# leochlon/aecf

Hardware: AMD Instinct MI355X
Metric: fused samples/sec (fwd+bwd) (higher is better)
Workload: dtype bf16; 1 GPU; c2: [B=65536 per GPU, M=3, d=512, 8 heads] mask_prob=0.15 train-mode curriculum masking, fwd+bwd; global_batch=65536, parallelism=dp1, world_size=1

## Files before the change

aecf_amd/csrc/aecf_gemm_ws.hip:

```cpp
#include <stdlib.h>

#include "aecf_kernels.h"
#include "aecf_tile.h"

namespace aecf {

namespace {

enum { WS_PLAIN = 0, WS_VPROJ = 1, WS_VFLAT = 2 };

constexpr int WS_PF = 3, VPROJ_PF = 3, DX_PF = 3;

constexpr int ws_plain_bufs(int, int) { return 2; }

template <int KT, int NROWS, int KEYDIV>
__device__ __forceinline__ void ws_dma_rows(const char* __restrict__ src, unsigned int ld_bytes, int rows_valid, char* lds) {
    constexpr int CPR = 4 * KT;
    constexpr int TOTAL = NROWS * CPR;
    constexpr int NI = (TOTAL + 511) / 512;
    static_assert(TOTAL % 64 == 0, "whole wave-instructions");
    const int wbase = __builtin_amdgcn_readfirstlane((int)(threadIdx.x & ~63u));
#pragma unroll
    for (int i = 0; i < NI; ++i) {
        if (wbase + 512 * i < TOTAL) {
            const int c = threadIdx.x + 512 * i;
            const int row = c / CPR, p = c - row * CPR;
            const int rowc = row < rows_valid ? row : rows_valid - 1;
            const int key = (row / KEYDIV) & 15;
            const unsigned int voff = (unsigned)rowc * ld_bytes + (unsigned)((p ^ key) << 4);
            __builtin_amdgcn_global_load_lds(src + voff, (lds_void_t*)(lds + (wbase + 512 * i) * 16), 16, 0, 0);
        }
    }
}

template <int CT>
__device__ __forceinline__ void store_packed(unsigned short* dst, const unsigned int* pk) {
    if (CT == 2) *reinterpret_cast<u32x4*>(dst) = u32x4{pk[0], pk[1], pk[2], pk[3]};
    else *reinterpret_cast<u32x2*>(dst) = u32x2{pk[0], pk[1]};
}
template <int CT>
__device__ __forceinline__ void store_cols_f32(float* dst, const float* v) {
    *reinterpret_cast<f32x4*>(dst) = f32x4{v[0], v[1], v[2], v[3]};
    if (CT == 2) *reinterpret_cast<f32x4*>(dst + 4) = f32x4{v[4], v[5], v[6], v[7]};
}
template <int CT>
__device__ __forceinline__ void store_cols(unsigned short* dst, const float* v);
template <int CT>
__device__ __forceinline__ void store_cols_lo(unsigned short* dst, const float* v) {
    float lo[4 * CT];
#pragma unroll
    for (int j = 0; j < 4 * CT; ++j) lo[j] = v[j] - Tr<BF16>::to_f32(Tr<BF16>::from_f32(v[j]));
    store_cols<CT>(dst, lo);
}
template <int CT>
__device__ __forceinline__ void store_cols(unsigned short* dst, const float* v) {
    if (CT == 2) {
        *reinterpret_cast<u32x4*>(dst) = u32x4{pack_bf16x2(v[0], v[1]), pack_bf16x2(v[2], v[3]), pack_bf16x2(v[4], v[5]),
// ... 10 lines not shown
    for (int m = 0; m < M_; ++m) {
        sc[m] = __builtin_amdgcn_exp2f((sc[m] - mx) * 1.44269504088896340736f);
        sum += sc[m];
    }
    float inv = __builtin_amdgcn_rcpf(sum);
    inv = inv * (2.0f - sum * inv);
#pragma unroll
    for (int m = 0; m < M_; ++m) sc[m] *= inv;
}

template <int NV>
__device__ __forceinline__ void load_bias(const unsigned short* bs, int col, float* bias) {
#pragma unroll
    for (int j = 0; j < NV; ++j) bias[j] = 0.f;
    if (bs) {
        if (NV == 8) {
            Tr<BF16>::unpack(*reinterpret_cast<const u32x4*>(bs + col), bias);
        } else {
            Tr<BF16>::load4(bs + col, bias);
        }
    }
}

template <int KT, int MODE, int M_, bool GATE, int CT>
__global__ __launch_bounds__(512, 2) void gemm_ws_kernel(GemmNtArgs p, int rows_per_block, int nchunk) {
    using X = Tr<BF16>;
    constexpr int K = 32 * KT, ROWB = 2 * K;
    constexpr bool PL = MODE != WS_VPROJ;
    constexpr bool VF = MODE == WS_VFLAT;
    constexpr int NPM = MODE == WS_VPROJ ? M_ : (VF ? 2 : 1);
    constexpr int RT = PL ? 2 : M_;
    constexpr int SROWS = 16 * RT;
    constexpr int OROWS = PL ? 32 : 16;
    constexpr int TILE = SROWS * ROWB;
    constexpr int NBUF = ws_plain_bufs(MODE, KT);
    constexpr int NI_DMA = SROWS * 4 * KT / 512;
    extern __shared__ __attribute__((aligned(16))) char smem[];

    const int lane = lane_id(), r16 = lane & 15, lg = lane >> 4, w = wave_id();
    const int N = p.N, H = p.H;
    unsigned int chunk_u, group_u;
    constexpr int CW = 16 * CT, BC = 8 * CW, NV = 4 * CT;
    if (!xcd_tile(blockIdx.x, (unsigned)nchunk, (unsigned)(p.N / BC), chunk_u, group_u)) return;
    const int ncol0 = (int)group_u * BC + CW * w;
    const int64_t o_beg = (int64_t)chunk_u * rows_per_block;
    const int64_t o_all = p.R;
    const int64_t o_end = (o_beg + rows_per_block) < o_all ? (o_beg + rows_per_block) : o_all;
// ... 21 lines not shown

    const unsigned short* wsrc = reinterpret_cast<const unsigned short*>(p.w);
    u32x4 wreg[KT][CT];
#pragma unroll
    for (int c = 0; c < CT; ++c) {
        const int n = CT == 2 ? ncol0 + 8 * (r16 >> 2) + 4 * c + (r16 & 3) : ncol0 + r16;
        const unsigned short* wr = wsrc + (int64_t)n * K + 8 * lg;
        const u32x4* wf = reinterpret_cast<const u32x4*>(p.w_frag) + ((int64_t)((ncol0 / CW) * CT + c) * KT) * 64 + lane;
#pragma unroll
        for (int ks = 0; ks < KT; ++ks) wreg[ks][c] = p.w_frag ? wf[ks * 64] : *reinterpret_cast<const u32x4*>(wr + 32 * ks);
    }
    float bias[NV];
    load_bias<NV>(reinterpret_cast<const unsigned short*>(p.bias), ncol0 + NV * lg, bias);
    const int head = ncol0 / p.hd;

    int xaddr[4];
#pragma unroll
    for (int v = 0; v < 4; ++v)
        xaddr[v] = (PL ? r16 : r16 * M_) * ROWB + ((((4 * v) + lg) ^ r16) << 4);

    float pm[NPM], pm_next[NPM];
    constexpr int KG = (KT + 7) / 8;
    float* gpart = reinterpret_cast<float*>(smem + 2 * TILE);
    u32x4 ga[GATE ? KG : 1][2];
    if (GATE) {
#pragma unroll
        for (int kg = 0; kg < KG; ++kg) {
            const int ks = KG * w + kg;
            const unsigned short* ah = reinterpret_cast<const unsigned short*>(p.g_ahi) + (int64_t)r16 * K + 32 * ks + 8 * lg;
            const unsigned short* al = reinterpret_cast<const unsigned short*>(p.g_alo) + (int64_t)r16 * K + 32 * ks + 8 * lg;
            ga[kg][0] = ks < KT ? *reinterpret_cast<const u32x4*>(ah) : u32x4{0u, 0u, 0u, 0u};
            ga[kg][1] = ks < KT ? *reinterpret_cast<const u32x4*>(al) : u32x4{0u, 0u, 0u, 0u};
        }
    }
    unsigned int kp[GATE ? M_ : 1], kp_next[GATE ? M_ : 1];
    auto load_probs = [&](int64_t o0, float* dst) {
        if (MODE == WS_VPROJ && GATE) {
            if (p.g_kpm) {
                const int64_t b = (o0 + r16) < o_end ? (o0 + r16) : (o_end - 1);
                const uint8_t* kq = p.g_kpm + b * M_;
#pragma unroll
                for (int m = 0; m < M_; ++m)
                    asm volatile("global_load_ubyte %0, %1, off" : "=v"(kp_next[m]) : "v"(kq + m) : "memory");
            }
        } else if (MODE == WS_VPROJ) {
            const int64_t b = (o0 + r16) < o_end ? (o0 + r16) : (o_end - 1);
            const float* pp = p.probs + (b * H + head) * M_;
#pragma unroll
            for (int m = 0; m < M_; ++m)
                asm volatile("global_load_dword %0, %1, off" : "=v"(dst[m]) : "v"(pp + m) : "memory");
        } else if (VF) {
#pragma unroll
            for (int t = 0; t < 2; ++t) {
                const int64_t row = (o0 + 16 * t + r16) < o_end ? (o0 + 16 * t + r16) : (o_end - 1);
// ... 10 lines not shown
        if (GATE) { asm volatile("" : "+v"(kp_next[m])); kp[m] = p.g_kpm ? kp_next[m] : 0u; }
        else asm volatile("" : "+v"(pm[m]));
    }
    int cur = 0;
    for (int64_t o0 = o_beg; o0 < o_end; o0 += OROWS, cur = (cur + 1 == NBUF ? 0 : cur + 1)) {
        __builtin_amdgcn_s_barrier();
        const bool two_ahead = NBUF == 3 && o0 + 2 * OROWS < o_end;
        if (NBUF == 3) { if (two_ahead) issue(o0 + 2 * OROWS, cur >= 1 ? cur - 1 : 2); }
        else if (!GATE && o0 + OROWS < o_end) issue(o0 + OROWS, cur ^ 1);
        if (o0 + OROWS < o_end) load_probs(o0 + OROWS, pm_next);

        if (GATE) {
            const char* tg = smem + cur * TILE;
            f32x4 gacc[M_];
#pragma unroll
            for (int m = 0; m < M_; ++m) {
                gacc[m] = f32x4{0.f, 0.f, 0.f, 0.f};
#pragma unroll
                for (int kg = 0; kg < KG; ++kg) {
                    const int ks = (KG * w + kg) % KT;
                    const int xo = r16 * M_ * ROWB + m * ROWB + ((((ks & 3) * 4 + lg) ^ r16) << 4) + (ks >> 2) * 256;
                    const u32x4 xf = *reinterpret_cast<const u32x4*>(tg + xo);
                    gacc[m] = X::mma(ga[kg][0], xf, gacc[m]);
                    gacc[m] = X::mma(ga[kg][1], xf, gacc[m]);
                }
#pragma unroll
                for (int r = 0; r < 4; ++r) gpart[((w * M_ + m) * 16 + 4 * lg + r) * 16 + r16] = gacc[m][r];
            }
            asm volatile("s_waitcnt lgkmcnt(0)" ::: "memory");
            __builtin_amdgcn_s_barrier();
            float sc[M_], mx = -INFINITY;
#pragma unroll
            for (int m = 0; m < M_; ++m) {
                float a = 0.f;
#pragma unroll
                for (int ww = 0; ww < 8; ++ww) a += gpart[((ww * M_ + m) * 16 + head) * 16 + r16];
                if (kp[m] != 0u) a = -INFINITY;
                sc[m] = a;
                mx = fmaxf(mx, a);
            }
            softmax_fast<M_>(sc, mx);
            const int64_t bq = o0 + r16;
            const bool writer = lg == 0 && ncol0 % p.hd == 0 && bq < o_end;
#pragma unroll
            for (int m = 0; m < M_; ++m) pm[m] = sc[m];
            if (writer) {
                float* dst = const_cast<float*>(p.probs) + (bq * H + head) * M_;
#pragma unroll
                for (int m = 0; m < M_; ++m) dst[m] = pm[m];
            }
        }

        constexpr int NIT = RT * KT;
        constexpr int PF = WS_PF;
        const char* tb = smem + cur * TILE;
        auto rd = [&](int i) -> u32x4 {
            const int ks = PL ? i / RT : i % KT;
            const int t = PL ? i % RT : i / KT;
            const int toff = (PL ? 16 * t * ROWB : t * ROWB) + (ks >> 2) * 256;
            return *reinterpret_cast<const u32x4*>(tb + xaddr[ks & 3] + toff);
        };
        constexpr int NACC = PL ? RT : 1;
        f32x4 acc[NACC][CT];
#pragma unroll
        for (int t = 0; t < NACC; ++t)
#pragma unroll
            for (int c = 0; c < CT; ++c) acc[t][c] = f32x4{0.f, 0.f, 0.f, 0.f};
        float ov[NV];
        unsigned int vpk[MODE == WS_VPROJ ? M_ : 1][NV / 2];
#pragma unroll
        for (int j = 0; j < NV; ++j) ov[j] = 0.f;

        u32x4 xf[PF + 1];
#pragma unroll
        for (int i = 0; i < PF; ++i) xf[i] = rd(i);
        __builtin_amdgcn_sched_group_barrier(0x100, PF, 0);
#pragma unroll
        for (int i = 0; i < NIT; ++i) {
            if (i + PF < NIT) xf[(i + PF) % (PF + 1)] = rd(i + PF);
            if (GATE && i == NIT / 8 && o0 + OROWS < o_end) issue(o0 + OROWS, cur ^ 1);
            const int ks = PL ? i / RT : i % KT;
            const int t = PL ? i % RT : 0;
#pragma unroll
            for (int c = 0; c < CT; ++c) acc[t][c] = X::mma(wreg[ks][c], xf[i % (PF + 1)], acc[t][c]);
            __builtin_amdgcn_sched_group_barrier(0x100, 1, 0);
            __builtin_amdgcn_sched_group_barrier(0x008, CT, 0);
            if (MODE == WS_VPROJ && ks == KT - 1) {
                const int m = i / KT;
                float v[NV];
#pragma unroll
                for (int c = 0; c < CT; ++c)
#pragma unroll
                    for (int r = 0; r < 4; ++r) {
                        v[4 * c + r] = acc[0][c][r] + bias[4 * c + r];
                        ov[4 * c + r] = fmaf(pm[m], v[4 * c + r], ov[4 * c + r]);
                    }
#pragma unroll
                for (int j = 0; j < NV / 2; ++j) vpk[m][j] = pack_bf16x2(v[2 * j], v[2 * j + 1]);
#pragma unroll
                for (int c = 0; c < CT; ++c) acc[0][c] = f32x4{0.f, 0.f, 0.f, 0.f};
            }
        }

        if (two_ahead) asm volatile("s_waitcnt vmcnt(%0)" ::"n"(NI_DMA) : "memory");
        else asm volatile("s_waitcnt vmcnt(0)" ::: "memory");
        float pm_now[NPM];
#pragma unroll
        for (int m = 0; m < NPM; ++m) pm_now[m] = pm[m];
#pragma unroll
        for (int m = 0; m < NPM; ++m) {
            if (GATE) {
                asm volatile("" : "+v"(kp_next[m]));
                kp[m] = p.g_kpm ? kp_next[m] : 0u;
            } else {
                asm volatile("" : "+v"(pm_next[m]));
                pm[m] = pm_next[m];
            }
        }
        if (PL) {
#pragma unroll
            for (int t = 0; t < RT; ++t) {
// ... 9 lines not shown
                        else store_cols<CT>(reinterpret_cast<unsigned short*>(p.c) + row * N + ncol0 + NV * lg, v);
                        if (p.c_lo) store_cols_lo<CT>(reinterpret_cast<unsigned short*>(p.c_lo) + row * N + ncol0 + NV * lg, v);
                    }
                } else {
                    if (p.v_out && row < o_end)
                        store_cols<CT>(reinterpret_cast<unsigned short*>(p.v_out) + row * N + ncol0 + NV * lg, v);
                    float ow[NV];
#pragma unroll
                    for (int j = 0; j < NV; ++j) {
                        float a = pm_now[t] * v[j];
                        a += __shfl_xor(a, 1, 64);
                        a += __shfl_xor(a, 2, 64);
                        ow[j] = a;
                    }
                    if ((r16 & 3) == 0 && row < o_end) {
                        store_cols<CT>(reinterpret_cast<unsigned short*>(p.c) + (row / M_) * N + ncol0 + NV * lg, ow);
                        if (p.c_lo) store_cols_lo<CT>(reinterpret_cast<unsigned short*>(p.c_lo) + (row / M_) * N + ncol0 + NV * lg, ow);
                    }
                }
            }
        } else {
            const int64_t b = o0 + r16;
            if (b < o_end) {
                if (p.v_out) {
#pragma unroll
                    for (int m = 0; m < M_; ++m)
                        store_packed<CT>(reinterpret_cast<unsigned short*>(p.v_out) + (b * M_ + m) * N + ncol0 + NV * lg, vpk[m]);
                }
                if (p.out_f32) store_cols_f32<CT>(reinterpret_cast<float*>(p.c) + b * N + ncol0 + NV * lg, ov);
                else store_cols<CT>(reinterpret_cast<unsigned short*>(p.c) + b * N + ncol0 + NV * lg, ov);
                if (p.c_lo) store_cols_lo<CT>(reinterpret_cast<unsigned short*>(p.c_lo) + b * N + ncol0 + NV * lg, ov);
            }
        }
    }
}

template <int KT, int HK, int M_, int CT>
__global__ __launch_bounds__(512, 2) void dx_ws2_kernel(BwdGArgs p, int rows_per_block, int nchunk) {
    using X = Tr<BF16>;
    constexpr int CW = 16 * CT, BC = 8 * CW, NV = 4 * CT;
    constexpr int K = 32 * KT, ROWB = 2 * K;
    constexpr int H_ = KT / HK;
    constexpr int KX = (3 * H_ + 31) / 32;
    constexpr int RAW = 16 * ROWB;
    constexpr int HM = H_ * M_, NST = 16 * HM;
    constexpr int HMS = HM | 1;
    extern __shared__ __attribute__((aligned(16))) char smem[];
    constexpr int XROWB = 64 * KX + 16;
    constexpr int XT = 16 * M_ * XROWB;
    char* raw = smem;
// ... 193 lines not shown
    }
}

template <int KT, int HK, int M_, bool HILO>
__global__ __launch_bounds__(512, 2) void dsu_ws_kernel(BwdGArgs p, float* __restrict__ u_slab, int rows_per_block, int nchunk) {
    using X = Tr<BF16>;
    constexpr int KJ = 8;
    constexpr int E = 32 * KT, JB = 32 * KJ, NCT = KT / 4;
    constexpr int HBL = KJ / HK;
    constexpr int ROWX = 2 * E, ROWD = 2 * JB;
    constexpr int XROWS = 16 * M_;
    constexpr int KU = (XROWS + 31) / 32;
    constexpr int ZROWS = (32 * KU - XROWS) > 0 ? 1 : 0;
    constexpr int PSTR = HBL * M_ * 16;
    constexpr int DSROW = 72;
    constexpr int XT = XROWS * ROWX, DT = 16 * ROWD;
    constexpr int NPART = 8;
    extern __shared__ __attribute__((aligned(16))) char smem[];
    char* xb = smem;
    char* zp = smem + 2 * XT;
    char* db = zp + ZROWS * ROWX;
    char* dbl = db + 2 * DT;
    float* part = reinterpret_cast<float*>(db + (HILO ? 4 : 2) * DT);
    unsigned short* dsh = reinterpret_cast<unsigned short*>(reinterpret_cast<char*>(part) + NPART * PSTR * 4);
    unsigned short* dsl = dsh + 16 * DSROW;

    const int lane = lane_id(), r16 = lane & 15, lg = lane >> 4;
    const int w = __builtin_amdgcn_readfirstlane(wave_id());
    const int H = p.H;
    unsigned int chunk_u, group_u;
    if (!xcd_tile(blockIdx.x, (unsigned)nchunk, (unsigned)(E / JB), chunk_u, group_u)) return;
    const int jbase = (int)group_u * JB, hbase = jbase / (32 * HK);
    const int ncol0 = 16 * NCT * w;
    const int64_t o_beg = (int64_t)chunk_u * rows_per_block;
    const int64_t o_end = (o_beg + rows_per_block) < p.B ? (o_beg + rows_per_block) : p.B;
    if (o_beg >= o_end) return;

    const char* dsrc = reinterpret_cast<const char*>(p.dobuf) + (int64_t)jbase * 2;
    const char* xsrc = reinterpret_cast<const char*>(p.x);
    const char* dlsrc = HILO ? reinterpret_cast<const char*>(p.do_lo) + (int64_t)jbase * 2 : dsrc;
    auto issue = [&](int64_t o0, int buf) {
        const int ov = (int)((o_end - o0) < 16 ? (o_end - o0) : 16);
        ws_dma_rows_asm<KT, 16 * M_, M_>(xsrc + o0 * M_ * (int64_t)ROWX, (unsigned)ROWX, ov * M_, xb + buf * XT);
        ws_dma_rows_asm<KJ, 16, 1>(dsrc + o0 * (int64_t)ROWX, (unsigned)ROWX, ov, db + buf * DT);
        if (HILO) ws_dma_rows_asm<KJ, 16, 1>(dlsrc + o0 * (int64_t)ROWX, (unsigned)ROWX, ov, dbl + buf * DT);
    };
    for (int i = threadIdx.x; i < ZROWS * ROWX / 16; i += 512) reinterpret_cast<u32x4*>(zp)[i] = u32x4{0u, 0u, 0u, 0u};
    for (int i = threadIdx.x; i < 2 * 16 * DSROW / 2; i += 512) reinterpret_cast<unsigned int*>(dsh)[i] = 0u;
    issue(o_beg, 0);

    const unsigned short* wsrc = reinterpret_cast<const unsigned short*>(p.wvt);
    u32x4 wreg[KJ][NCT];
    static_assert(NCT % 2 == 0, "tile pairs");
#pragma unroll
    for (int ct = 0; ct < NCT; ++ct) {
        const int krow = ncol0 + 32 * (ct >> 1) + 8 * (r16 >> 2) + 4 * (ct & 1) + (r16 & 3);
        const unsigned short* wr = wsrc + (int64_t)krow * E + jbase + 8 * lg;
#pragma unroll
        for (int ks = 0; ks < KJ; ++ks) wreg[ks][ct] = *reinterpret_cast<const u32x4*>(wr + 32 * ks);
    }
    int daddr[4];
#pragma unroll
    for (int v = 0; v < 4; ++v) daddr[v] = r16 * ROWD + ((((4 * v) + lg) ^ r16) << 4);
    const int xaddr0 = r16 * M_ * ROWX + ((((ncol0 >> 3) + lg) ^ r16) << 4);
    const int q = r16 >> 2, pp = r16 & 3;
    int ua[KU][2];
    bool uz[KU][2];
#pragma unroll
    for (int ks = 0; ks < KU; ++ks) {
#pragma unroll
        for (int hh = 0; hh < 2; ++hh) {
// ... 102 lines not shown
            if (ds_m < M_) {
                const float* pr = part + (ds_hh * M_ + ds_m) * 16 + ds_s;
#pragma unroll
                for (int i = 0; i < NPART; ++i) da += pr[i * PSTR];
            }
            float dw = p.d_attn_w ? dwb : 0.f;
            if (p.d_entropy && ds_m < M_) {
                int64_t be = o0 + ds_s;
                be = be < o_end ? be : o_end - 1;
                float hsum = 0.f;
#pragma unroll
                for (int m = 0; m < M_; ++m) hsum -= xlogx(p.attn_w[be * M_ + m]);
                const bool live = (hsum >= 0.f) && (hsum <= p.log_M);
                dw += live ? -(logf(p.attn_w[be * M_ + ds_m]) + 1.0f) * p.d_entropy[be] : 0.f;
            }
            const float dp = da + dw * invH;
            const float dot = reduce_lg((ds_m < M_) ? pmv * dp : 0.f);
            const int64_t b = o0 + ds_s;
            if (ds_m < M_) {
                const float d = (b < o_end) ? pmv * (dp - dot) : 0.f;
                if (b < o_end) p.dsbuf[(b * H + hbase + ds_hh) * M_ + ds_m] = d;
                const unsigned short hi = X::from_f32(d);
                dsh[ds_hh * DSROW + kslot(ds_s, ds_m)] = hi;
                dsl[ds_hh * DSROW + kslot(ds_s, ds_m)] = X::from_f32(d - X::to_f32(hi));
            }
        }
        asm volatile("s_waitcnt lgkmcnt(0)" ::: "memory");
        __builtin_amdgcn_s_barrier();
#pragma unroll
        for (int ks = 0; ks < KU; ++ks) {
            const u32x4 bh = *reinterpret_cast<const u32x4*>(reinterpret_cast<const char*>(dsh) + (r16 * DSROW + 32 * ks + 8 * lg) * 2);
            const u32x4 bl = *reinterpret_cast<const u32x4*>(reinterpret_cast<const char*>(dsl) + (r16 * DSROW + 32 * ks + 8 * lg) * 2);
#pragma unroll
            for (int ct = 0; ct < NCT; ++ct) {
                const u32x4 af = tr_frag16(smem, (uz[ks][0] ? 0 : cur * XT) + (ua[ks][0] ^ (32 * ct)),
                                           (uz[ks][1] ? 0 : cur * XT) + (ua[ks][1] ^ (32 * ct)));
                uacc[ct] = X::mma(af, bh, uacc[ct]);
                uacc[ct] = X::mma(af, bl, uacc[ct]);
            }
        }
        asm volatile("s_waitcnt vmcnt(0)" ::: "memory");
        asm volatile("" : "+v"(pmv_n), "+v"(dwb_n));
        pmv = pmv_n; dwb = dwb_n;
    }
    if (r16 < HBL) {
#pragma unroll
        for (int ct = 0; ct < NCT; ++ct)
            *reinterpret_cast<f32x4*>(u_slab + ((int64_t)chunk_u * H + hbase + r16) * E + ncol0 + 16 * ct + 4 * lg) = uacc[ct];
    }
}


static size_t dsu_ws_smem(int E, int M, int hd, bool lo) {
    constexpr int JB = 256;
    const int xrows = 16 * M, zrows = (32 * ((xrows + 31) / 32) - xrows) > 0 ? 1 : 0, hbl = JB / hd;
    return (size_t)(2 * xrows + zrows) * 2 * E + (size_t)(lo ? 4 : 2) * 16 * 2 * JB + (size_t)8 * (16 * hbl * M) * 4 +
           (size_t)2 * 16 * 72 * 2;
}

template <int KT, int HK, int M_>
int launch_dsu_t(const BwdGArgs& a, float* u_slab, hipStream_t s) {
    constexpr int E = 32 * KT, JB = 256;
    const bool hilo = a.do_lo && dsu_ws_takes_lo(a);
    const size_t smem = dsu_ws_smem(E, M_, a.hd, hilo);
    const int groups = E / JB;
    int64_t chunks = 256 / groups;
    if (chunks < 1) chunks = 1;
    int64_t rpb = (a.B + chunks - 1) / chunks;
    rpb = (rpb + 15) / 16 * 16;
    const int64_t nchunk = (a.B + rpb - 1) / rpb;
    dim3 grid(xcd_grid((unsigned)nchunk, (unsigned)groups)), block(512);
    if constexpr (!(E == 512 && M_ == 4)) {
        if (hilo) {
            auto kern = dsu_ws_kernel<KT, HK, M_, true>;
            (void)hipFuncSetAttribute(reinterpret_cast<const void*>(kern), hipFuncAttributeMaxDynamicSharedMemorySize, (int)smem);
            kern<<<grid, block, smem, s>>>(a, u_slab, (int)rpb, (int)nchunk);
            return (int)nchunk;
        }
    }
    auto kern = dsu_ws_kernel<KT, HK, M_, false>;
// ... 30 lines not shown
        default: launch_dx2<KT, HK, 4>(a, s); break;
    }
}

template <int KT>
bool launch_dx2_hk(const BwdGArgs& a, hipStream_t s) {
    static_assert(KT % 8 == 0 && KT <= 32, "K = 256, 512, 768, 1024");
    const int hk = a.hd / 32;
    if (hk * a.H != KT) return false;
    if constexpr (KT <= 16) {
        if (hk == 1) { launch_dx2_m<KT, 1>(a, s); return true; }
    }
    if (hk == 2) { launch_dx2_m<KT, 2>(a, s); return true; }
    if constexpr (KT % 3 == 0) {
        if (hk == 3) { launch_dx2_m<KT, 3>(a, s); return true; }
    }
    if (hk == 4) { launch_dx2_m<KT, 4>(a, s); return true; }
    if (hk == 8) { launch_dx2_m<KT, 8>(a, s); return true; }
    if (hk == KT) { launch_dx2_m<KT, KT>(a, s); return true; }
    return false;
}


template <int M_>
__global__ __launch_bounds__(512, 2) void vproj_slab_kernel(GemmNtArgs p, int rows_per_block, int nchunk) {
    using X = Tr<BF16>;
    constexpr int KT = 16, K = 512, CT = 2, KG = 2;
    constexpr int SB = 128;
    constexpr int SLAB = 16 * M_ * SB;
    constexpr int TILE = 8 * SLAB;
    constexpr int CW = 32, BC = 256, NV = 8;
    constexpr int GP = 8 * M_ * 256;
    constexpr int NDMA = 16 * M_ * SB / 1024;
    extern __shared__ __attribute__((aligned(16))) char smem[];
    float* gpart = reinterpret_cast<float*>(smem + 2 * TILE);

    const int lane = lane_id(), r16 = lane & 15, lg = lane >> 4;
    const int w = __builtin_amdgcn_readfirstlane(wave_id());
    const int N = p.N, H = p.H;
    unsigned int chunk_u, group_u;
    if (!xcd_tile(blockIdx.x, (unsigned)nchunk, (unsigned)(p.N / BC), chunk_u, group_u)) return;
    const int ncol0 = (int)group_u * BC + CW * w;
    const int64_t o_beg = (int64_t)chunk_u * rows_per_block;
    const int64_t o_end = (o_beg + rows_per_block) < p.R ? (o_beg + rows_per_block) : p.R;
    if (o_beg >= o_end) return;

    const char* asrc = reinterpret_cast<const char*>(p.a);
    const unsigned int row_pitch = (unsigned)K * 2u;
    auto issue_piece = [&](int64_t o0, int buf, int i) {
        const int ov = (int)((o_end - o0) < 16 ? (o_end - o0) : 16);
        const char* src = asrc + o0 * M_ * (int64_t)row_pitch + SB * w;
        const int rho = 8 * i + (lane >> 3), m = rho >> 4, b = rho & 15;
        const int bc = b < ov ? b : ov - 1;
        const unsigned int voff = (unsigned)(bc * M_ + m) * row_pitch + (unsigned)(((lane & 7) ^ (b & 7)) << 4);
        const unsigned int dst = (unsigned)(size_t)(lds_void_t*)(smem + buf * TILE + w * SLAB + 1024 * i);
// ... 6 lines not shown
    auto issue = [&](int64_t o0, int buf) {
#pragma unroll
        for (int i = 0; i < NDMA; ++i) issue_piece(o0, buf, i);
    };
    issue(o_beg, 0);

    const unsigned short* wsrc = reinterpret_cast<const unsigned short*>(p.w);
    u32x4 wreg[KT][CT];
#pragma unroll
    for (int c = 0; c < CT; ++c) {
        const int n = ncol0 + 8 * (r16 >> 2) + 4 * c + (r16 & 3);
        const unsigned short* wr = wsrc + (int64_t)n * K + 8 * lg;
        const u32x4* wf = reinterpret_cast<const u32x4*>(p.w_frag) + ((int64_t)((ncol0 / CW) * CT + c) * KT) * 64 + lane;
#pragma unroll
        for (int ks = 0; ks < KT; ++ks) wreg[ks][c] = p.w_frag ? wf[ks * 64] : *reinterpret_cast<const u32x4*>(wr + 32 * ks);
    }
    float bias[NV];
    load_bias<NV>(reinterpret_cast<const unsigned short*>(p.bias), ncol0 + NV * lg, bias);
    const int head = ncol0 / p.hd;
    int xoff[KG];
#pragma unroll
    for (int kk = 0; kk < KG; ++kk) xoff[kk] = r16 * SB + ((((4 * kk) + lg) ^ (r16 & 7)) << 4);

    u32x4 ga[KG][2];
#pragma unroll
    for (int kg = 0; kg < KG; ++kg) {
        const int ks = KG * w + kg;
        ga[kg][0] = *reinterpret_cast<const u32x4*>(reinterpret_cast<const unsigned short*>(p.g_ahi) + (int64_t)r16 * K + 32 * ks + 8 * lg);
        ga[kg][1] = *reinterpret_cast<const u32x4*>(reinterpret_cast<const unsigned short*>(p.g_alo) + (int64_t)r16 * K + 32 * ks + 8 * lg);
    }
    unsigned int kp[M_], kp_next[M_];
    {
        const int64_t b0 = (o_beg + r16) < o_end ? (o_beg + r16) : (o_end - 1);
#pragma unroll
        for (int m = 0; m < M_; ++m) {
            kp[m] = p.g_kpm ? (unsigned int)p.g_kpm[b0 * M_ + m] : 0u;
            kp_next[m] = 0u;
        }
    }
    auto load_kp = [&](int64_t o0) {
        if (p.g_kpm) {
            const int64_t b = (o0 + r16) < o_end ? (o0 + r16) : (o_end - 1);
            const uint8_t* kq = p.g_kpm + b * M_;
#pragma unroll
            for (int m = 0; m < M_; ++m) asm volatile("global_load_ubyte %0, %1, off" : "+v"(kp_next[m]) : "v"(kq + m) : "memory");
        }
    };
    auto scores = [&](int buf, float* gp) {
        const char* sl = smem + buf * TILE + w * SLAB;
#pragma unroll
        for (int m = 0; m < M_; ++m) {
            f32x4 gacc = f32x4{0.f, 0.f, 0.f, 0.f};
#pragma unroll
            for (int kg = 0; kg < KG; ++kg) {
                const u32x4 xf = *reinterpret_cast<const u32x4*>(sl + m * 16 * SB + xoff[kg]);
                gacc = X::mma(ga[kg][0], xf, gacc);
                gacc = X::mma(ga[kg][1], xf, gacc);
            }
#pragma unroll
            for (int r = 0; r < 4; ++r) gp[((w * M_ + m) * 16 + 4 * lg + r) * 16 + r16] = gacc[r];
        }
    };
#pragma unroll
    for (int ks = 0; ks < KT; ++ks)
#pragma unroll
        for (int c = 0; c < CT; ++c) asm volatile("" : "+v"(wreg[ks][c]));
#pragma unroll
    for (int kg = 0; kg < KG; ++kg) asm volatile("" : "+v"(ga[kg][0]), "+v"(ga[kg][1]));
    asm volatile("s_waitcnt vmcnt(0)" ::: "memory");
    scores(0, gpart);

    int cur = 0;
    for (int64_t o0 = o_beg; o0 < o_end; o0 += 16, cur ^= 1) {
        const bool more = o0 + 16 < o_end;
        asm volatile("s_waitcnt lgkmcnt(0)" ::: "memory");
        __builtin_amdgcn_s_barrier();
        if (more) load_kp(o0 + 16);
        float pm[M_];
        {
            const float* gp = gpart + cur * GP;
            float mx = -INFINITY;
#pragma unroll
            for (int m = 0; m < M_; ++m) {
                float a = 0.f;
#pragma unroll
                for (int ww = 0; ww < 8; ++ww) a += gp[((ww * M_ + m) * 16 + head) * 16 + r16];
                if (kp[m] != 0u) a = -INFINITY;
                pm[m] = a;
                mx = fmaxf(mx, a);
            }
            softmax_fast<M_>(pm, mx);
            const int64_t bq = o0 + r16;
            const bool writer = lg == 0 && ncol0 % p.hd == 0 && bq < o_end;
            if (writer) {
                float* dst = const_cast<float*>(p.probs) + (bq * H + head) * M_;
#pragma unroll
                for (int m = 0; m < M_; ++m) dst[m] = pm[m];
            }
        }
        constexpr int NIT = M_ * KT, PF = VPROJ_PF;
        const char* tb = smem + cur * TILE;
        auto rd = [&](int i) -> u32x4 {
            const int ks = i % KT, m = i / KT;
            return *reinterpret_cast<const u32x4*>(tb + (ks >> 1) * SLAB + m * 16 * SB + xoff[ks & 1]);
        };
        f32x4 acc[CT];
#pragma unroll
        for (int c = 0; c < CT; ++c) acc[c] = f32x4{0.f, 0.f, 0.f, 0.f};
        float ov[NV];
        unsigned int vpk[M_][NV / 2];
#pragma unroll
        for (int j = 0; j < NV; ++j) ov[j] = 0.f;
        u32x4 xf[PF + 1];
#pragma unroll
        for (int i = 0; i < PF; ++i) xf[i] = rd(i);
        __builtin_amdgcn_sched_group_barrier(0x100, PF, 0);
#pragma unroll
        for (int i = 0; i < NIT; ++i) {
            if (i + PF < NIT) xf[(i + PF) % (PF + 1)] = rd(i + PF);
            if (i == NIT / 8 && more) issue(o0 + 16, cur ^ 1);
            const int ks = i % KT;
#pragma unroll
            for (int c = 0; c < CT; ++c) acc[c] = X::mma(wreg[ks][c], xf[i % (PF + 1)], acc[c]);
            __builtin_amdgcn_sched_group_barrier(0x100, 1, 0);
            __builtin_amdgcn_sched_group_barrier(0x008, CT, 0);
            if (ks == KT - 1) {
                const int m = i / KT;
                float v[NV];
#pragma unroll
                for (int c = 0; c < CT; ++c)
#pragma unroll
                    for (int r = 0; r < 4; ++r) {
                        v[4 * c + r] = acc[c][r] + bias[4 * c + r];
                        ov[4 * c + r] = fmaf(pm[m], v[4 * c + r], ov[4 * c + r]);
                    }
#pragma unroll
                for (int j = 0; j < NV / 2; ++j) vpk[m][j] = pack_bf16x2(v[2 * j], v[2 * j + 1]);
#pragma unroll
                for (int c = 0; c < CT; ++c) acc[c] = f32x4{0.f, 0.f, 0.f, 0.f};
            }
        }
        asm volatile("s_waitcnt vmcnt(0)" ::: "memory");
#pragma unroll
        for (int m = 0; m < M_; ++m) { asm volatile("" : "+v"(kp_next[m])); kp[m] = p.g_kpm ? kp_next[m] : 0u; }
        if (more) scores(cur ^ 1, gpart + (cur ^ 1) * GP);
        const int64_t b = o0 + r16;
        if (b < o_end) {
            if (p.v_out) {
#pragma unroll
                for (int m = 0; m < M_; ++m)
                    store_packed<CT>(reinterpret_cast<unsigned short*>(p.v_out) + (b * M_ + m) * N + ncol0 + NV * lg, vpk[m]);
            }
            if (p.out_f32) store_cols_f32<CT>(reinterpret_cast<float*>(p.c) + b * N + ncol0 + NV * lg, ov);
            else store_cols<CT>(reinterpret_cast<unsigned short*>(p.c) + b * N + ncol0 + NV * lg, ov);
            if (p.c_lo) store_cols_lo<CT>(reinterpret_cast<unsigned short*>(p.c_lo) + b * N + ncol0 + NV * lg, ov);
        }
    }
}

template <int M_>
void launch_vproj_slab(const GemmNtArgs& a, hipStream_t s) {
    const size_t smem = (size_t)2 * 16 * M_ * 1024 + (size_t)2 * 8 * M_ * 256 * sizeof(float);
    const int groups = a.N / 256;
    int64_t chunks = 256 / groups;
    if (chunks < 1) chunks = 1;
    int64_t rpb = (a.R + chunks - 1) / chunks;
    rpb = (rpb + 15) / 16 * 16;
    const int64_t nchunk = (a.R + rpb - 1) / rpb;
    dim3 grid(xcd_grid((unsigned)nchunk, (unsigned)groups)), block(512);
    auto kern = vproj_slab_kernel<M_>;
    (void)hipFuncSetAttribute(reinterpret_cast<const void*>(kern), hipFuncAttributeMaxDynamicSharedMemorySize, (int)smem);
    kern<<<grid, block, smem, s>>>(a, (int)rpb, (int)nchunk);
}

template <int KT, int MODE, int M_, bool GATE>
void launch_ws(const GemmNtArgs& a, hipStream_t s) {
    constexpr int K = 32 * KT;
    constexpr int CT = KT <= 16 ? 2 : 1;
    constexpr int RT = MODE != WS_VPROJ ? 2 : M_;
    constexpr int OROWS = MODE != WS_VPROJ ? 32 : 16;
    size_t smem = (size_t)ws_plain_bufs(MODE, KT) * 16 * RT * 2 * K;
    const int groups = a.N / (128 * CT);
    int64_t chunks = 256 / groups;
    if (chunks < 1) chunks = 1;
    int64_t rpb = (a.R + chunks - 1) / chunks;
    rpb = (rpb + OROWS - 1) / OROWS * OROWS;
    const int64_t nchunk = (a.R + rpb - 1) / rpb;
    dim3 grid(xcd_grid((unsigned)nchunk, (unsigned)groups)), block(512);
    if (GATE) smem += (size_t)8 * M_ * 256 * sizeof(float);
    auto kern = gemm_ws_kernel<KT, MODE, M_, GATE, CT>;
    if (smem > 64 * 1024)
        (void)hipFuncSetAttribute(reinterpret_cast<const void*>(kern), hipFuncAttributeMaxDynamicSharedMemorySize, (int)smem);
    kern<<<grid, block, smem, s>>>(a, (int)rpb, (int)nchunk);
}

constexpr bool ws_built(int KT, int MODE, int M, bool gate) {
    if (MODE == WS_PLAIN) return true;
    if (KT == 4 || KT == 12) return false;
    if (MODE == WS_VFLAT) return KT >= 24;
    if (M == 4) return KT <= 16;
    return 2 * 16 * M * 2 * 32 * KT + (gate ? 8 * M * 1024 : 0) <= 150 * 1024;
}

template <int MODE, int M_, bool GATE>
void launch_kt(const GemmNtArgs& a, hipStream_t s) {
    switch (a.K / 32) {
        case 4: if constexpr (ws_built(4, MODE, M_, GATE)) launch_ws<4, MODE, M_, GATE>(a, s); break;
        case 8: if constexpr (ws_built(8, MODE, M_, GATE)) launch_ws<8, MODE, M_, GATE>(a, s); break;
        case 12: if constexpr (ws_built(12, MODE, M_, GATE)) launch_ws<12, MODE, M_, GATE>(a, s); break;
        case 16:
            if constexpr (GATE) launch_vproj_slab<M_>(a, s);
            else if constexpr (ws_built(16, MODE, M_, GATE)) launch_ws<16, MODE, M_, GATE>(a, s);
            break;
        case 24: if constexpr (ws_built(24, MODE, M_, GATE)) launch_ws<24, MODE, M_, GATE>(a, s); break;
        default: if constexpr (ws_built(32, MODE, M_, GATE)) launch_ws<32, MODE, M_, GATE>(a, s); break;
    }
}

}

static bool ws_k_ok(int K) { return K == 128 || K == 256 || K == 384 || K == 512 || K == 768 || K == 1024; }

static bool ws_vproj_flat(const GemmNtArgs& a) {
    const size_t tile = (size_t)16 * a.M * 2 * a.K;
    return (a.pooled & 1) && a.M == 4 && !a.g_ahi && 2 * tile > 150 * 1024 && (size_t)2 * 32 * 2 * a.K <= 150 * 1024;
}

bool gemm_ws_supported(const GemmNtArgs& a) {
    if (!ws_k_ok(a.K)) return false;
    if (a.out_f32 && (a.pooled & 1) && ws_vproj_flat(a)) return false;
    const int ct = a.K <= 512 ? 2 : 1;
    if (a.N % (128 * ct) != 0) return false;
    const bool vproj = (a.pooled & 1) != 0;
    if (vproj && ws_vproj_flat(a)) return a.hd % (16 * ct) == 0 && a.lda == (int64_t)a.M * a.K;
    const size_t tile = (size_t)16 * (vproj ? a.M : 2) * 2 * a.K;
    size_t smem = 2 * tile + (vproj && a.g_ahi ? (size_t)8 * a.M * 1024 : 0);
    if (smem > 150 * 1024) return false;
    if (vproj) return a.M >= 1 && a.M <= 4 && a.hd % 32 == 0 && a.lda == (int64_t)a.M * a.K;
    return a.lda == a.K;
}

void launch_gemm_ws(const GemmNtArgs& a, hipStream_t s) {
    if (ws_vproj_flat(a)) {
        GemmNtArgs f = a;
        f.R = a.R * a.M;
        f.lda = a.K;
        launch_kt<WS_VFLAT, 4, false>(f, s);
        return;
    }
    if (a.pooled & 1) {
        switch (a.M) {
            case 1: if (a.g_ahi) launch_kt<WS_VPROJ, 1, true>(a, s); else launch_kt<WS_VPROJ, 1, false>(a, s); break;
            case 2: if (a.g_ahi) launch_kt<WS_VPROJ, 2, true>(a, s); else launch_kt<WS_VPROJ, 2, false>(a, s); break;
            case 3: if (a.g_ahi) launch_kt<WS_VPROJ, 3, true>(a, s); else launch_kt<WS_VPROJ, 3, false>(a, s); break;
            default: launch_kt<WS_VPROJ, 4, false>(a, s); break;
        }
    } else {
        launch_kt<WS_PLAIN, 1, false>(a, s);
    }
// ... 61 lines not shown
```

Baseline: 119.8 million samples/s.

## Pack hi/lo gate split into one MFMA and skip unused V stores

When the head count is at most 8, the gate scoring packs hi and lo A-operand rows into the two halves of one 16-row MFMA. This halves the gate MFMAs, and the halves are combined with a permlane32 swap. The gate partial layout becomes padded per-head rows, and the softmax reads one value per lane then spreads it with permlane swaps instead of M strided LDS reductions. The backward dscore GEMM likewise stores hi/lo rows together in one tile, drops the second MFMA and reduces with a shuffle. A VOUT template flag removes the packing and storing of per-modality V outputs when v_out is null. The added lane shuffles and new template variants add complexity and carry some risk of layout mistakes.

Result: faster. 121.3 million samples/s, median of 5 (+1.2%).

```diff
diff --git a/aecf_amd/csrc/aecf_gemm_ws.hip b/aecf_amd/csrc/aecf_gemm_ws.hip
--- a/aecf_amd/csrc/aecf_gemm_ws.hip
+++ b/aecf_amd/csrc/aecf_gemm_ws.hip
@@ -33,6 +33,23 @@
     }
 }
 
+constexpr int gate_hs(int M) { return 16 * M + 4; }
+constexpr int gate_part_floats(int M, int NH) { return 8 * NH * gate_hs(M); }
+
+template <int M_>
+__device__ __forceinline__ void gate_share(float a, float* sc) {
+    const unsigned int u = __float_as_uint(a);
+    const auto h = __builtin_amdgcn_permlane32_swap(u, u, false, false);
+    const auto lo = __builtin_amdgcn_permlane16_swap(h[0], h[0], false, false);
+    sc[0] = __uint_as_float(lo[0]);
+    if (M_ > 1) sc[M_ > 1 ? 1 : 0] = __uint_as_float(lo[1]);
+    if (M_ > 2) {
+        const auto hi = __builtin_amdgcn_permlane16_swap(h[1], h[1], false, false);
+        sc[M_ > 2 ? 2 : 0] = __uint_as_float(hi[0]);
+        if (M_ > 3) sc[M_ > 3 ? 3 : 0] = __uint_as_float(hi[1]);
+    }
+}
+
 template <int CT>
 __device__ __forceinline__ void store_packed(unsigned short* dst, const unsigned int* pk) {
     if (CT == 2) *reinterpret_cast<u32x4*>(dst) = u32x4{pk[0], pk[1], pk[2], pk[3]};
@@ -89,7 +106,7 @@
     }
 }
 
-template <int KT, int MODE, int M_, bool GATE, int CT>
+template <int KT, int MODE, int M_, bool GATE, int CT, bool VOUT>
 __global__ __launch_bounds__(512, 2) void gemm_ws_kernel(GemmNtArgs p, int rows_per_block, int nchunk) {
     using X = Tr<BF16>;
     constexpr int K = 32 * KT, ROWB = 2 * K;
@@ -157,14 +174,16 @@
     float pm[NPM], pm_next[NPM];
     constexpr int KG = (KT + 7) / 8;
     float* gpart = reinterpret_cast<float*>(smem + 2 * TILE);
+    constexpr int HS = gate_hs(M_);
+    const bool pack = H <= 8;
     u32x4 ga[GATE ? KG : 1][2];
     if (GATE) {
 #pragma unroll
         for (int kg = 0; kg < KG; ++kg) {
             const int ks = KG * w + kg;
             const unsigned short* ah = reinterpret_cast<const unsigned short*>(p.g_ahi) + (int64_t)r16 * K + 32 * ks + 8 * lg;
-            const unsigned short* al = reinterpret_cast<const unsigned short*>(p.g_alo) + (int64_t)r16 * K + 32 * ks + 8 * lg;
-            ga[kg][0] = ks < KT ? *reinterpret_cast<const u32x4*>(ah) : u32x4{0u, 0u, 0u, 0u};
+            const unsigned short* al = reinterpret_cast<const unsigned short*>(p.g_alo) + (int64_t)(pack ? r16 & 7 : r16) * K + 32 * ks + 8 * lg;
+            ga[kg][0] = ks < KT ? *reinterpret_cast<const u32x4*>(pack && r16 >= 8 ? al : ah) : u32x4{0u, 0u, 0u, 0u};
             ga[kg][1] = ks < KT ? *reinterpret_cast<const u32x4*>(al) : u32x4{0u, 0u, 0u, 0u};
         }
     }
@@ -221,22 +240,34 @@
                     const int xo = r16 * M_ * ROWB + m * ROWB + ((((ks & 3) * 4 + lg) ^ r16) << 4) + (ks >> 2) * 256;
                     const u32x4 xf = *reinterpret_cast<const u32x4*>(tg + xo);
                     gacc[m] = X::mma(ga[kg][0], xf, gacc[m]);
-                    gacc[m] = X::mma(ga[kg][1], xf, gacc[m]);
+                    if (!pack) gacc[m] = X::mma(ga[kg][1], xf, gacc[m]);
                 }
-#pragma unroll
-                for (int r = 0; r < 4; ++r) gpart[((w * M_ + m) * 16 + 4 * lg + r) * 16 + r16] = gacc[m][r];
+                if (pack) {
+#pragma unroll
+                    for (int r = 0; r < 4; ++r) {
+                        const unsigned int u = __float_as_uint(gacc[m][r]);
+                        const auto sw = __builtin_amdgcn_permlane32_swap(u, u, false, false);
+                        gacc[m][r] = __uint_as_float(sw[0]) + __uint_as_float(sw[1]);
+                    }
+                }
+                const int hrow = pack ? 4 * (lg & 1) : 4 * lg;
+#pragma unroll
+                for (int r = 0; r < 4; ++r) gpart[(w * 16 + hrow + r) * HS + m * 16 + r16] = gacc[m][r];
             }
             asm volatile("s_waitcnt lgkmcnt(0)" ::: "memory");
             __builtin_amdgcn_s_barrier();
             float sc[M_], mx = -INFINITY;
+            {
+                const float* gq = gpart + head * HS + (lg < M_ ? lg : M_ - 1) * 16 + r16;
+                float a = 0.f;
+#pragma unroll
+                for (int ww = 0; ww < 8; ++ww) a += gq[ww * 16 * HS];
+                gate_share<M_>(a, sc);
+            }
 #pragma unroll
             for (int m = 0; m < M_; ++m) {
-                float a = 0.f;
-#pragma unroll
-                for (int ww = 0; ww < 8; ++ww) a += gpart[((ww * M_ + m) * 16 + head) * 16 + r16];
-                if (kp[m] != 0u) a = -INFINITY;
-                sc[m] = a;
-                mx = fmaxf(mx, a);
+                if (kp[m] != 0u) sc[m] = -INFINITY;
+                mx = fmaxf(mx, sc[m]);
             }
             softmax_fast<M_>(sc, mx);
             const int64_t bq = o0 + r16;
@@ -266,7 +297,8 @@
 #pragma unroll
             for (int c = 0; c < CT; ++c) acc[t][c] = f32x4{0.f, 0.f, 0.f, 0.f};
         float ov[NV];
-        unsigned int vpk[MODE == WS_VPROJ ? M_ : 1][NV / 2];
+        constexpr bool VPK = MODE == WS_VPROJ && VOUT;
+        unsigned int vpk[VPK ? M_ : 1][NV / 2];
 #pragma unroll
         for (int j = 0; j < NV; ++j) ov[j] = 0.f;
 
@@ -294,8 +326,10 @@
                         v[4 * c + r] = acc[0][c][r] + bias[4 * c + r];
                         ov[4 * c + r] = fmaf(pm[m], v[4 * c + r], ov[4 * c + r]);
                     }
-#pragma unroll
-                for (int j = 0; j < NV / 2; ++j) vpk[m][j] = pack_bf16x2(v[2 * j], v[2 * j + 1]);
+                if (VPK) {
+#pragma unroll
+                    for (int j = 0; j < NV / 2; ++j) vpk[VPK ? m : 0][j] = pack_bf16x2(v[2 * j], v[2 * j + 1]);
+                }
 #pragma unroll
                 for (int c = 0; c < CT; ++c) acc[0][c] = f32x4{0.f, 0.f, 0.f, 0.f};
             }
@@ -351,10 +385,10 @@
         } else {
             const int64_t b = o0 + r16;
             if (b < o_end) {
-                if (p.v_out) {
+                if (VPK && p.v_out) {
 #pragma unroll
                     for (int m = 0; m < M_; ++m)
-                        store_packed<CT>(reinterpret_cast<unsigned short*>(p.v_out) + (b * M_ + m) * N + ncol0 + NV * lg, vpk[m]);
+                        store_packed<CT>(reinterpret_cast<unsigned short*>(p.v_out) + (b * M_ + m) * N + ncol0 + NV * lg, vpk[VPK ? m : 0]);
                 }
                 if (p.out_f32) store_cols_f32<CT>(reinterpret_cast<float*>(p.c) + b * N + ncol0 + NV * lg, ov);
                 else store_cols<CT>(reinterpret_cast<unsigned short*>(p.c) + b * N + ncol0 + NV * lg, ov);
@@ -594,8 +628,8 @@
     char* db = zp + ZROWS * ROWX;
     char* dbl = db + 2 * DT;
     float* part = reinterpret_cast<float*>(db + (HILO ? 4 : 2) * DT);
+    static_assert(HBL <= 8, "hi and lo rows side by side");
     unsigned short* dsh = reinterpret_cast<unsigned short*>(reinterpret_cast<char*>(part) + NPART * PSTR * 4);
-    unsigned short* dsl = dsh + 16 * DSROW;
 
     const int lane = lane_id(), r16 = lane & 15, lg = lane >> 4;
     const int w = __builtin_amdgcn_readfirstlane(wave_id());
@@ -618,7 +652,7 @@
         if (HILO) ws_dma_rows_asm<KJ, 16, 1>(dlsrc + o0 * (int64_t)ROWX, (unsigned)ROWX, ov, dbl + buf * DT);
     };
     for (int i = threadIdx.x; i < ZROWS * ROWX / 16; i += 512) reinterpret_cast<u32x4*>(zp)[i] = u32x4{0u, 0u, 0u, 0u};
-    for (int i = threadIdx.x; i < 2 * 16 * DSROW / 2; i += 512) reinterpret_cast<unsigned int*>(dsh)[i] = 0u;
+    for (int i = threadIdx.x; i < 16 * DSROW / 2; i += 512) reinterpret_cast<unsigned int*>(dsh)[i] = 0u;
     issue(o_beg, 0);
 
     const unsigned short* wsrc = reinterpret_cast<const unsigned short*>(p.wvt);
@@ -767,7 +801,7 @@
                 if (b < o_end) p.dsbuf[(b * H + hbase + ds_hh) * M_ + ds_m] = d;
                 const unsigned short hi = X::from_f32(d);
                 dsh[ds_hh * DSROW + kslot(ds_s, ds_m)] = hi;
-                dsl[ds_hh * DSROW + kslot(ds_s, ds_m)] = X::from_f32(d - X::to_f32(hi));
+                dsh[(8 + ds_hh) * DSROW + kslot(ds_s, ds_m)] = X::from_f32(d - X::to_f32(hi));
             }
         }
         asm volatile("s_waitcnt lgkmcnt(0)" ::: "memory");
@@ -775,19 +809,21 @@
 #pragma unroll
         for (int ks = 0; ks < KU; ++ks) {
             const u32x4 bh = *reinterpret_cast<const u32x4*>(reinterpret_cast<const char*>(dsh) + (r16 * DSROW + 32 * ks + 8 * lg) * 2);
-            const u32x4 bl = *reinterpret_cast<const u32x4*>(reinterpret_cast<const char*>(dsl) + (r16 * DSROW + 32 * ks + 8 * lg) * 2);
 #pragma unroll
             for (int ct = 0; ct < NCT; ++ct) {
                 const u32x4 af = tr_frag16(smem, (uz[ks][0] ? 0 : cur * XT) + (ua[ks][0] ^ (32 * ct)),
                                            (uz[ks][1] ? 0 : cur * XT) + (ua[ks][1] ^ (32 * ct)));
                 uacc[ct] = X::mma(af, bh, uacc[ct]);
-                uacc[ct] = X::mma(af, bl, uacc[ct]);
             }
         }
         asm volatile("s_waitcnt vmcnt(0)" ::: "memory");
         asm volatile("" : "+v"(pmv_n), "+v"(dwb_n));
         pmv = pmv_n; dwb = dwb_n;
     }
+#pragma unroll
+    for (int ct = 0; ct < NCT; ++ct)
+#pragma unroll
+        for (int r = 0; r < 4; ++r) uacc[ct][r] += __shfl_down(uacc[ct][r], 8, 64);
     if (r16 < HBL) {
 #pragma unroll
         for (int ct = 0; ct < NCT; ++ct)
@@ -800,7 +836,7 @@
     constexpr int JB = 256;
     const int xrows = 16 * M, zrows = (32 * ((xrows + 31) / 32) - xrows) > 0 ? 1 : 0, hbl = JB / hd;
     return (size_t)(2 * xrows + zrows) * 2 * E + (size_t)(lo ? 4 : 2) * 16 * 2 * JB + (size_t)8 * (16 * hbl * M) * 4 +
-           (size_t)2 * 16 * 72 * 2;
+           (size_t)16 * 72 * 2;
 }
 
 template <int KT, int HK, int M_>
@@ -877,15 +913,16 @@
 }
 
 
-template <int M_>
+template <int M_, bool PACK, bool VOUT>
 __global__ __launch_bounds__(512, 2) void vproj_slab_kernel(GemmNtArgs p, int rows_per_block, int nchunk) {
     using X = Tr<BF16>;
     constexpr int KT = 16, K = 512, CT = 2, KG = 2;
+    constexpr int NH = PACK ? 8 : 16, HS = gate_hs(M_);
     constexpr int SB = 128;
     constexpr int SLAB = 16 * M_ * SB;
     constexpr int TILE = 8 * SLAB;
     constexpr int CW = 32, BC = 256, NV = 8;
-    constexpr int GP = 8 * M_ * 256;
+    constexpr int GP = gate_part_floats(M_, NH);
     constexpr int NDMA = 16 * M_ * SB / 1024;
     extern __shared__ __attribute__((aligned(16))) char smem[];
     float* gpart = reinterpret_cast<float*>(smem + 2 * TILE);
@@ -938,12 +975,15 @@
 #pragma unroll
     for (int kk = 0; kk < KG; ++kk) xoff[kk] = r16 * SB + ((((4 * kk) + lg) ^ (r16 & 7)) << 4);
 
-    u32x4 ga[KG][2];
+    constexpr int NGA = PACK ? 1 : 2;
+    u32x4 ga[KG][NGA];
 #pragma unroll
     for (int kg = 0; kg < KG; ++kg) {
         const int ks = KG * w + kg;
-        ga[kg][0] = *reinterpret_cast<const u32x4*>(reinterpret_cast<const unsigned short*>(p.g_ahi) + (int64_t)r16 * K + 32 * ks + 8 * lg);
-        ga[kg][1] = *reinterpret_cast<const u32x4*>(reinterpret_cast<const unsigned short*>(p.g_alo) + (int64_t)r16 * K + 32 * ks + 8 * lg);
+        const unsigned short* ah = reinterpret_cast<const unsigned short*>(p.g_ahi) + (int64_t)r16 * K + 32 * ks + 8 * lg;
+        const unsigned short* al = reinterpret_cast<const unsigned short*>(p.g_alo) + (int64_t)(PACK ? r16 & 7 : r16) * K + 32 * ks + 8 * lg;
+        ga[kg][0] = *reinterpret_cast<const u32x4*>(PACK && r16 >= 8 ? al : ah);
+        if (!PACK) ga[kg][NGA - 1] = *reinterpret_cast<const u32x4*>(al);
     }
     unsigned int kp[M_], kp_next[M_];
     {
@@ -971,10 +1011,19 @@
             for (int kg = 0; kg < KG; ++kg) {
                 const u32x4 xf = *reinterpret_cast<const u32x4*>(sl + m * 16 * SB + xoff[kg]);
                 gacc = X::mma(ga[kg][0], xf, gacc);
-                gacc = X::mma(ga[kg][1], xf, gacc);
-            }
-#pragma unroll
-            for (int r = 0; r < 4; ++r) gp[((w * M_ + m) * 16 + 4 * lg + r) * 16 + r16] = gacc[r];
+                if (!PACK) gacc = X::mma(ga[kg][NGA - 1], xf, gacc);
+            }
+            if (PACK) {
+#pragma unroll
+                for (int r = 0; r < 4; ++r) {
+                    const unsigned int u = __float_as_uint(gacc[r]);
+                    const auto sw = __builtin_amdgcn_permlane32_swap(u, u, false, false);
+                    gacc[r] = __uint_as_float(sw[0]) + __uint_as_float(sw[1]);
+                }
+            }
+            const int hrow = PACK ? 4 * (lg & 1) : 4 * lg;
+#pragma unroll
+            for (int r = 0; r < 4; ++r) gp[(w * NH + hrow + r) * HS + m * 16 + r16] = gacc[r];
         }
     };
 #pragma unroll
@@ -982,7 +1031,7 @@
 #pragma unroll
         for (int c = 0; c < CT; ++c) asm volatile("" : "+v"(wreg[ks][c]));
 #pragma unroll
-    for (int kg = 0; kg < KG; ++kg) asm volatile("" : "+v"(ga[kg][0]), "+v"(ga[kg][1]));
+    for (int kg = 0; kg < KG; ++kg) asm volatile("" : "+v"(ga[kg][0]), "+v"(ga[kg][NGA - 1]));
     asm volatile("s_waitcnt vmcnt(0)" ::: "memory");
     scores(0, gpart);
 
@@ -994,16 +1043,16 @@
         if (more) load_kp(o0 + 16);
         float pm[M_];
         {
-            const float* gp = gpart + cur * GP;
+            const float* gq = gpart + cur * GP + head * HS + (lg < M_ ? lg : M_ - 1) * 16 + r16;
+            float a = 0.f;
+#pragma unroll
+            for (int ww = 0; ww < 8; ++ww) a += gq[ww * NH * HS];
+            gate_share<M_>(a, pm);
             float mx = -INFINITY;
 #pragma unroll
             for (int m = 0; m < M_; ++m) {
-                float a = 0.f;
-#pragma unroll
-                for (int ww = 0; ww < 8; ++ww) a += gp[((ww * M_ + m) * 16 + head) * 16 + r16];
-                if (kp[m] != 0u) a = -INFINITY;
-                pm[m] = a;
-                mx = fmaxf(mx, a);
+                if (kp[m] != 0u) pm[m] = -INFINITY;
+                mx = fmaxf(mx, pm[m]);
             }
             softmax_fast<M_>(pm, mx);
             const int64_t bq = o0 + r16;
@@ -1024,7 +1073,7 @@
 #pragma unroll
         for (int c = 0; c < CT; ++c) acc[c] = f32x4{0.f, 0.f, 0.f, 0.f};
         float ov[NV];
-        unsigned int vpk[M_][NV / 2];
+        unsigned int vpk[VOUT ? M_ : 1][NV / 2];
 #pragma unroll
         for (int j = 0; j < NV; ++j) ov[j] = 0.f;
         u32x4 xf[PF + 1];
@@ -1050,8 +1099,10 @@
                         v[4 * c + r] = acc[c][r] + bias[4 * c + r];
                         ov[4 * c + r] = fmaf(pm[m], v[4 * c + r], ov[4 * c + r]);
                     }
-#pragma unroll
-                for (int j = 0; j < NV / 2; ++j) vpk[m][j] = pack_bf16x2(v[2 * j], v[2 * j + 1]);
+                if (VOUT) {
+#pragma unroll
+                    for (int j = 0; j < NV / 2; ++j) vpk[VOUT ? m : 0][j] = pack_bf16x2(v[2 * j], v[2 * j + 1]);
+                }
 #pragma unroll
                 for (int c = 0; c < CT; ++c) acc[c] = f32x4{0.f, 0.f, 0.f, 0.f};
             }
@@ -1062,10 +1113,10 @@
         if (more) scores(cur ^ 1, gpart + (cur ^ 1) * GP);
         const int64_t b = o0 + r16;
         if (b < o_end) {
-            if (p.v_out) {
+            if (VOUT && p.v_out) {
 #pragma unroll
                 for (int m = 0; m < M_; ++m)
-                    store_packed<CT>(reinterpret_cast<unsigned short*>(p.v_out) + (b * M_ + m) * N + ncol0 + NV * lg, vpk[m]);
+                    store_packed<CT>(reinterpret_cast<unsigned short*>(p.v_out) + (b * M_ + m) * N + ncol0 + NV * lg, vpk[VOUT ? m : 0]);
             }
             if (p.out_f32) store_cols_f32<CT>(reinterpret_cast<float*>(p.c) + b * N + ncol0 + NV * lg, ov);
             else store_cols<CT>(reinterpret_cast<unsigned short*>(p.c) + b * N + ncol0 + NV * lg, ov);
@@ -1074,9 +1125,9 @@
     }
 }
 
-template <int M_>
-void launch_vproj_slab(const GemmNtArgs& a, hipStream_t s) {
-    const size_t smem = (size_t)2 * 16 * M_ * 1024 + (size_t)2 * 8 * M_ * 256 * sizeof(float);
+template <int M_, bool PACK, bool VOUT>
+void launch_vproj_slab_t(const GemmNtArgs& a, hipStream_t s) {
+    const size_t smem = (size_t)2 * 16 * M_ * 1024 + (size_t)2 * gate_part_floats(M_, PACK ? 8 : 16) * sizeof(float);
     const int groups = a.N / 256;
     int64_t chunks = 256 / groups;
     if (chunks < 1) chunks = 1;
@@ -1084,9 +1135,16 @@
     rpb = (rpb + 15) / 16 * 16;
     const int64_t nchunk = (a.R + rpb - 1) / rpb;
     dim3 grid(xcd_grid((unsigned)nchunk, (unsigned)groups)), block(512);
-    auto kern = vproj_slab_kernel<M_>;
+    auto kern = vproj_slab_kernel<M_, PACK, VOUT>;
     (void)hipFuncSetAttribute(reinterpret_cast<const void*>(kern), hipFuncAttributeMaxDynamicSharedMemorySize, (int)smem);
     kern<<<grid, block, smem, s>>>(a, (int)rpb, (int)nchunk);
+}
+
+template <int M_>
+void launch_vproj_slab(const GemmNtArgs& a, hipStream_t s) {
+    if (a.H > 8) launch_vproj_slab_t<M_, false, true>(a, s);
+    else if (a.v_out) launch_vproj_slab_t<M_, true, true>(a, s);
+    else launch_vproj_slab_t<M_, true, false>(a, s);
 }
 
 template <int KT, int MODE, int M_, bool GATE>
@@ -1103,11 +1161,16 @@
     rpb = (rpb + OROWS - 1) / OROWS * OROWS;
     const int64_t nchunk = (a.R + rpb - 1) / rpb;
     dim3 grid(xcd_grid((unsigned)nchunk, (unsigned)groups)), block(512);
-    if (GATE) smem += (size_t)8 * M_ * 256 * sizeof(float);
-    auto kern = gemm_ws_kernel<KT, MODE, M_, GATE, CT>;
-    if (smem > 64 * 1024)
-        (void)hipFuncSetAttribute(reinterpret_cast<const void*>(kern), hipFuncAttributeMaxDynamicSharedMemorySize, (int)smem);
-    kern<<<grid, block, smem, s>>>(a, (int)rpb, (int)nchunk);
+    if (GATE) smem += (size_t)gate_part_floats(M_, 16) * sizeof(float);
+    auto launch = [&](auto kern) {
+        if (smem > 64 * 1024)
+            (void)hipFuncSetAttribute(reinterpret_cast<const void*>(kern), hipFuncAttributeMaxDynamicSharedMemorySize, (int)smem);
+        kern<<<grid, block, smem, s>>>(a, (int)rpb, (int)nchunk);
+    };
+    if constexpr (MODE == WS_VPROJ) {
+        if (!a.v_out) { launch(gemm_ws_kernel<KT, MODE, M_, GATE, CT, false>); return; }
+    }
+    launch(gemm_ws_kernel<KT, MODE, M_, GATE, CT, true>);
 }
 
 constexpr bool ws_built(int KT, int MODE, int M, bool gate) {
@@ -1115,7 +1178,7 @@
     if (KT == 4 || KT == 12) return false;
     if (MODE == WS_VFLAT) return KT >= 24;
     if (M == 4) return KT <= 16;
-    return 2 * 16 * M * 2 * 32 * KT + (gate ? 8 * M * 1024 : 0) <= 150 * 1024;
+    return 2 * 16 * M * 2 * 32 * KT + (gate ? gate_part_floats(M, 16) * 4 : 0) <= 150 * 1024;
 }
 
 template <int MODE, int M_, bool GATE>
@@ -1150,7 +1213,7 @@
     const bool vproj = (a.pooled & 1) != 0;
     if (vproj && ws_vproj_flat(a)) return a.hd % (16 * ct) == 0 && a.lda == (int64_t)a.M * a.K;
     const size_t tile = (size_t)16 * (vproj ? a.M : 2) * 2 * a.K;
-    size_t smem = 2 * tile + (vproj && a.g_ahi ? (size_t)8 * a.M * 1024 : 0);
+    size_t smem = 2 * tile + (vproj && a.g_ahi ? (size_t)gate_part_floats(a.M, 16) * 4 : 0);
     if (smem > 150 * 1024) return false;
     if (vproj) return a.M >= 1 && a.M <= 4 && a.hd % 32 == 0 && a.lda == (int64_t)a.M * a.K;
     return a.lda == a.K;
```
